# twosigma/Cook

Hardware: AMD Instinct MI355X
Metric: match-cycles/sec at 1M pending x 50k offers (higher is better)
Workload: dtype f64

## Files before the change

cook_amd/csrc/classfit_host.hpp:

```cpp

static int classfit_env() {
  static const int v = [] {
    const char* s = std::getenv("COOK_CLASSFIT");
    return s && (s[0] == '0' || s[0] == '1') ? s[0] - '0' : -1;
  }();
  return v;
}
static bool classfit_by_default(const cook_engine* e) {
  const int f = classfit_env();
  if (f >= 0) return f == 1;
  return g_engines_on_device[e->device & 63].load() >= 6;
}
static size_t cf_lds_bytes_host(unsigned NP, unsigned M, bool eq, unsigned G, unsigned S) {
  size_t n = sizeof(CfFixed) + (size_t)NP * 10u;
  n = (n + 7u) & ~(size_t)7u;
  if (eq) n += (size_t)M * 8u;
  n += ((size_t)G + 1u) * 2u + (size_t)G * 2u + (size_t)S * 2u;
  return n + 64u;
}
bool cf_setup(cook_engine* e, const MatchIn& in, const MatchIn* in_dev, const MatchState& st, const JobRec* jr, const JobCons* jcons, const OfferA* oa, const OfferB* ob,
              CfPoolCtx& ctx) {
  const unsigned K = in.K, M = in.M, G = in.G;
  e->cf_inelig = 0x10000u;
  if (K == 0 || M == 0 || M > CF_SORT_N || G > CF_MAXG || in.good_enough < 1.0 || in.has_x || in.reserved_bits || in.host_dup) return false;
  if (e->cf_max_host == 0xFFFFFFFFu || (size_t)e->cf_max_host > 8u * (size_t)M + 65536u) return false;
  CfBuf b{};
  b.ctl = e->cf_ctl.ensure(1);
  b.jr = jr, b.jcons = jcons, b.oa = oa, b.ob = ob;
  b.attr8 = e->cf_attr8.ensure(M);
  b.max_host = e->cf_max_host;
  b.h2o = e->cf_h2o.ensure((size_t)b.max_host + 1u);
  b.pos_fc = e->cf_pos[0].ensure(M), b.pos_fm = e->cf_pos[1].ensure(M), b.pos_cid = e->cf_pos[2].ensure(M);
  b.scr_fc = e->cf_scr[0].ensure(M), b.scr_fm = e->cf_scr[1].ensure(M), b.scr_cid = e->cf_scr[2].ensure(M);
  b.jobs = e->cf_jobs.ensure(K);
  b.gcount = e->cf_gcount.ensure(std::max(1u, G));
  b.gmem = e->cf_gmem.ensure((size_t)std::max(1u, G) * CF_GMEM);
  static_assert(sizeof(CfCtl) % 4 == 0, "cf_init clears the control block word by word");
  KM<cf_init, 256>(e, "cf_init", std::min(div_up(b.max_host + 1u, 1024u), 512u), b, b.max_host + 1u, std::max(1u, G));
  KM<cf_scan, 256>(e, "cf_scan", div_up(std::max(K, M), 256), in_dev, b, K, M);
  KM<cf_prepare, 1024>(e, "cf_prepare", 1u, in_dev, b, st.jmin, K, M, G, in.host_dup, in.reserved_bits ? 1u : 0u);
  KM<cf_pack_jobs, 256>(e, "cf_pack_jobs", div_up(K, 256), in_dev, b, K);
  static_assert(offsetof(CfCtl, t) <= 512, "the control block's head is read back through the 512-byte scratch");
  pinned_copy(e, e->h_scratch, b.ctl, offsetof(CfCtl, t), hipMemcpyDeviceToHost);
  sync(e);
  CfCtl hc;
  std::memcpy((void*)&hc, e->h_scratch, offsetof(CfCtl, t));
  e->cf_inelig = hc.inelig;
  if (hc.inelig) return false;
  const unsigned NP = (M + 63u) & ~63u;
  const unsigned S = hc.any_group ? e->cf_group_run_total + hc.n_grouped : 0u;
  if (cf_lds_bytes_host(NP, M, hc.any_eq != 0u, hc.any_group ? G : 0u, S) > CF_LDS_BYTES || S > 60000u) {
    e->cf_inelig = CF_X_SHAPE;
    return false;
  }
  ctx.in = in_dev;
  ctx.st = st;
  ctx.b = b;
  return true;
}
static void cf_prof_print(const uint32_t* q) {
#ifdef CF_PROF
  std::fprintf(stderr, "CFPROF (x16 shader cycles) decider: slow steps %u (candidates %u evaluation %u commit %u) plain steps %u in %u walk-total %u | class wave 1: poll %u answer %u answers %u idle %u idles %u | class wave 2: poll %u answer %u answers %u idle %u idles %u | walk ticks(100MHz) %u | batch boundaries: decider %u, batches without a walked job %u\n", q[27], q[24], q[25], q[26], q[28], q[29], q[31], q[32], q[33], q[35], q[36], q[37], q[40], q[41], q[43], q[44], q[45], q[CFS_TICKS_WALK], q[30], q[38]);
  std::fprintf(stderr, "CFPROF plain steps %u, C++ steps %u; steps that left the plain form: gpu kind %u, novel hosts %u, group %u, answer missing after the re-reads %u, guard band %u, epoch end %u\n", q[46], q[47], q[34] & 65535u, q[34] >> 16, q[39] & 65535u, q[39] >> 16, q[42] & 65535u, q[42] >> 16);
#else
  (void)q;
#endif
}
void cf_run(cook_engine* lead, cook_engine* const* es, unsigned n, hipStream_t stream) {
  cook_engine* e = lead;
  for (unsigned i0 = 0; i0 < n; i0 += (unsigned)CF_PACK) {
    const unsigned c = std::min<unsigned>(CF_PACK, n - i0);
    CfPack pk{};
    for (unsigned x = 0; x < (unsigned)CF_PACK; ++x) pk.c[x] = es[i0 + (x < c ? x : 0u)]->placement.walk;
    KLS("cf_walk", stream, cf_walk, c, CF_THREADS, pk);
  }
  for (unsigned i = 0; i < n; ++i) {
    const CfPoolCtx& c = es[i]->placement.walk;
    const unsigned G = es[i]->last_in.G;
    if (G) KLS("cf_group_chains", stream, cf_group_chains, div_up(G, 256), 256, c.b, c.st, G);
  }
  constexpr size_t SLOT = 16 + 48 * 4;
  if (!lead->h_cf) COOK_HIP(hipHostMalloc((void**)&lead->h_cf, 64 * SLOT, hipHostMallocDefault));
  for (unsigned i = 0; i < n; ++i) {
    char* slot = lead->h_cf + i * SLOT;
    COOK_HIP(hipMemcpyAsync(slot, es[i]->placement.walk.st.summary, 16, hipMemcpyDeviceToHost, stream));
    COOK_HIP(hipMemcpyAsync(slot + 16, es[i]->placement.walk.b.ctl->stats, 48 * 4, hipMemcpyDeviceToHost, stream));
  }
  COOK_HIP(hipStreamSynchronize(stream));
  for (unsigned i = 0; i < n; ++i) {
    cook_engine* x = es[i];
    const unsigned* sum = (const unsigned*)(lead->h_cf + i * SLOT);
    if (sum[3] == 0xDEADu) lead->fail(COOK_E_STATE, "cf_walk: the pool's tables do not fit the workgroup's LDS (the host's check let it through)");
    std::memcpy(x->cf_stats, lead->h_cf + i * SLOT + 16, 48 * 4);
    cf_prof_print(x->cf_stats);
    WinCtl c{};
    c.matched = sum[0], c.head_matched = sum[1], c.rounds = sum[2], c.head = x->last_in.K, c.visited_sum = x->cf_stats[CFS_WALKED];
    c.t_seq = x->cf_stats[CFS_TICKS_TOTAL], c.t_setup = x->cf_stats[CFS_TICKS_PROLOGUE];
    x->placement_complete(3, c);
  }
}
```

cook_amd/csrc/classfit_walk.hpp:

```cpp
#pragma once
#if defined(CF_PROF) && !defined(CF_STATS)
#define CF_STATS 1
#endif
#ifdef CF_STATS
#define CF_STAT(x) x
#define CF_TICKS() cook_ticks()
#else
#define CF_STAT(x) ((void)0)
#define CF_TICKS() 0ull
#endif
#ifdef CF_PROF
#define CF_PROF_T(x) const unsigned long long x = __builtin_readcyclecounter()
#define CF_PROF_ADD(i, d) prof[i] += (unsigned long long)(d)
#define CF_PROF_WHY(n) why = why == 3u ? (n) : why
#define CF_PROF_LEAVE() (why < 4u ? leave_a += 1ull << (16u * why) : leave_b += 1ull << (16u * (why - 4u)))
#else
#define CF_PROF_T(x) ((void)0)
#define CF_PROF_ADD(i, d) ((void)0)
#define CF_PROF_WHY(n) ((void)0)
#define CF_PROF_LEAVE() ((void)0)
#endif

#ifndef CF_AHEAD
#define CF_AHEAD 10
#endif
constexpr unsigned CF_BOARD = CF_AHEAD;
#ifndef CF_SLOTS_N
#define CF_SLOTS_N 12
#endif
constexpr unsigned CF_SLOTS = CF_SLOTS_N;
static_assert(CF_BOARD + 2u <= CF_SLOTS, "a slot is free again before its wave writes it two rows on");
static_assert(CF_SLOTS == 12u || CF_SLOTS == 24u, "cf_slot and classfit_asm.hpp know these two");
static __device__ __forceinline__ unsigned cf_slot(unsigned ord) { return ord - CF_SLOTS * ((ord * 43u) >> (CF_SLOTS == 12u ? 9 : 10)); }
constexpr unsigned CF_OVL = 58;
constexpr unsigned CF_EPOCH_AT = COOK_SHAPE(58, 8);
constexpr unsigned CFW_BOOKS = 4;
enum : unsigned { CFM_EXACT = 1u, CFM_EPOCH = 2u, CFM_BATCH_END = 3u };
enum : unsigned { CFX_NEXT_BASE = 0, CFX_SPARE1, CFX_LOGN, CFX_LOG_APPLIED, CFX_WALK_LO, CFX_WALK_HI, CFX_EX_LANE, CFX_FMAX_LO, CFX_FMAX_HI, CFX_EPOCH, CFX_MATCH_LO, CFX_MATCH_HI,
                  CFX_B1_LO, CFX_B1_HI, CFX_OVN, CFX_MINFC, CFX_MINFM, CFX_N = 24 };
constexpr uint32_t CF_ENT_NONE = 0x80000000u, CF_ENT_AMB = 0x40000000u;

struct __attribute__((aligned(8))) CfFree {
  uint32_t c, m;
};
struct CfEnt {
  uint32_t tag, pad, pos, cid;
  uint32_t fc, fm;
  double fa;
};
struct CfLog {
  uint32_t info, pos;
  uint32_t ofc, ofm, nfc, nfm, pad0, pad1;
};
struct CfPost {
  double fa;
  uint32_t w0;
  uint32_t pos;
  uint32_t fc, fm, cls, aux;
};
struct CfJobU {
  unsigned c, m, kind, L, n_eq, n_nov, grouped, grp, eq0, eq1, nov0, nov1;
};
struct CfLds {
  CfFree* fcm;
  uint16_t* cid;
  CfEnt* board;
  CfLog* log;
  uint32_t* ctrl;
  uint64_t* attr8;
  uint16_t *goff, *gcnt, *gids;
  CfJob* ring;
  CfPost* post2;
  CfClass* cls;
  uint32_t* pw;
  uint32_t* aw;
  uint32_t* gk;
  uint32_t* ovt;
  uint32_t* ovl;
  uint32_t* ckept;
  uint32_t* misc;
  const uint32_t* t;
  const uint32_t* envw;
};

struct CfLv8 {
  uint32_t v0, v1, v2, v3, v4, v5, v6, v7;
};
#define CF_FOR8(F) F(0) F(1) F(2) F(3) F(4) F(5) F(6) F(7)
static __device__ __forceinline__ unsigned cf_level_of(const uint32_t* t, uint32_t fc) {
  unsigned n = 0;
#pragma unroll
// ... 269 lines not shown
  constexpr bool is_decider = ROLE == 0, is_class_wave = ROLE == 1, is_books = ROLE == 2;
  const unsigned tid = threadIdx.x, lane = lane_id();
  CfCtl* ctl = b.ctl;
  const unsigned K = wave_uniform_u32(S.envw[CFE_K]), cmin = wave_uniform_u32(S.envw[CFE_CMIN]), mmin = wave_uniform_u32(S.envw[CFE_MMIN]);
  const uint32_t* t = S.t;
  CfLv8 tl = CfLv8{0u, 0u, 0u, 0u, 0u, 0u, 0u, 0u};
  if (is_class_wave) tl = cf_levels_load(t);
#define n_cls wave_uniform_u32(S.envw[CFE_NCLS])
#define n_kind wave_uniform_u32(S.envw[CFE_NKIND])
#define NP wave_uniform_u32(S.envw[CFE_NP])
  CfChunkLane c;
  unsigned nch_wave = 0;
  cf_setup_chunks(S.cls, n_cls, is_class_wave ? lw : 0xFFu, lane, c, nch_wave);
  c.lv = CfLv8{0u, 0u, 0u, 0u, 0u, 0u, 0u, 0u}, c.la = c.lv;
  unsigned my_kinds = 0;
  {
    const unsigned forw = is_class_wave ? lw : (is_decider && lane >= CF_OVL ? lane - CF_OVL + 1u : 0xFFu);
    for (unsigned ci = 0; ci < n_cls; ++ci)
      if (S.cls[ci].wave == forw && S.cls[ci].kind < 32u) my_kinds |= 1u << S.cls[ci].kind;
  }
  const unsigned wk = is_class_wave ? wave_uniform_u32(my_kinds) : 0u;
  unsigned one_cls = 0xFFFFFFFFu, u_off = 0, u_n = 0;
  double u_hTc = 0.0, u_hTm = 0.0;
  auto class_setup = [&] {
    unsigned cnt = 0, ci0 = 0;
    for (unsigned ci = 0; ci < n_cls; ++ci)
      if (S.cls[ci].wave == lw) ++cnt, ci0 = ci;
    one_cls = cnt == 1u ? ci0 : 0xFFFFFFFFu;
    const CfClass* cl = &S.cls[ci0];
    u_off = cl->off, u_n = cl->n, u_hTc = cl->hTc, u_hTm = cl->hTm;
  };
  if (is_class_wave) {
    class_setup();
    for (unsigned ch = 0; ch < nch_wave; ++ch) cf_tighten(S, tl, lane, ch, c);
    if (rep == 0u && lw != 0u) cf_wave_tables(S, lw, lane, c, wk, n_kind);
  }
  CfOvLane o;
  o.valid = 0u, o.id = 0u, o.cls = 0u, o.fc = 0u, o.fm = 0u, o.hTc = 0.0, o.hTm = 0.0;
  unsigned nrm = 0, rm1 = 0xFFFFFFFFu, rm2 = 0xFFFFFFFFu;
  unsigned minfc_all = wave_uniform_u32(S.envw[CFE_MINFC]), minfm_all = wave_uniform_u32(S.envw[CFE_MINFM]);
  unsigned matched = 0, head = 0;
  unsigned jc = 0, jm = 0, jmeta = 0, jgrp = 0, jeq0 = 0, jeq1 = 0, jnov0 = 0, jnov1 = 0;
  int res = -1;
  unsigned long long b1m = 0ull;
  unsigned seen = 0, gen = 0;
  unsigned tight_applied = 0;
  bool bk_room0 = false, nx_room0 = false, nx_walk = false;
  unsigned st_scans = 0, st_exact = 0, st_open = 0, st_ovwin = 0, st_gpu = 0, st_epochs = 0, st_tight = 0, st_walked = 0, st_dead = 0, st_opendead = 0, st_spins = 0, st_flips = 0,
           st_rewinds = 0;
  unsigned long long tk_epoch = 0, tk_books = 0, tk_walk = 0, tk_phase1 = 0;
#ifdef CF_PROF
  unsigned long long prof[8] = {0, 0, 0, 0, 0, 0, 0, 0}, bnd0 = 0ull;
  unsigned long long leave_a = 0ull, leave_b = 0ull;
#endif
  auto job_of = [&](unsigned s) -> CfJobU {
    CfJobU J;
    J.c = (unsigned)wave_read_lane((int)jc, (int)s), J.m = (unsigned)wave_read_lane((int)jm, (int)s);
    const unsigned meta = (unsigned)wave_read_lane((int)jmeta, (int)s);
    J.kind = meta & 255u, J.L = (meta >> 8) & 15u, J.n_eq = (meta >> 12) & 15u, J.n_nov = (meta >> 16) & 15u, J.grouped = (meta >> 20) & 1u;
    J.grp = 0u, J.eq0 = J.eq1 = 0u, J.nov0 = J.nov1 = 0xFFFFFFFFu;
    if (meta >> 12) {
      J.grp = (unsigned)wave_read_lane((int)jgrp, (int)s), J.eq0 = (unsigned)wave_read_lane((int)jeq0, (int)s), J.eq1 = (unsigned)wave_read_lane((int)jeq1, (int)s),
      J.nov0 = (unsigned)wave_read_lane((int)jnov0, (int)s), J.nov1 = (unsigned)wave_read_lane((int)jnov1, (int)s);
    }
    return J;
  };
  auto tables_room_any = [&](unsigned L, unsigned m) -> bool {
    bool r = S.ovt[L] > m;
    for (unsigned x = 1; x <= (unsigned)CF_CW; ++x) r = r || S.aw[x * CF_LV + L] > m;
    return r;
  };
  auto tables_walk = [&](unsigned kind, unsigned L, unsigned m) -> bool {
    bool r = false;
    if (kind == 0u) {
      r = S.ovt[L] > m;
      for (unsigned x = 1; x <= (unsigned)CF_CW; ++x) r = r || S.pw[x * CF_LV + L] > m;
    } else if (kind < (unsigned)CF_MAXKIND) {
      r = S.gk[kind * CF_LV + L] > m;
    }
    return r;
  };
  CfJob nxt;
  nxt.c = nxt.m = nxt.meta = nxt.grp = nxt.eq[0] = nxt.eq[1] = nxt.nov[0] = nxt.nov[1] = 0u;
  constexpr unsigned CF_PRE = 3;
  CfJob pre[CF_PRE];
  auto books_next = [&](unsigned nbase) -> unsigned long long {
    const unsigned nn = nbase < K ? cf_min(64u, K - nbase) : 0u;
    const unsigned nslot = (nbase >> 6) & 1u;
    const bool in = lane < nn;
    if (in) S.ring[nslot * 64u + lane] = nxt;
    const unsigned kind = nxt.meta & 255u, L = (nxt.meta >> 8) & 15u;
    nx_room0 = in && tables_room_any(L, nxt.m);
    nx_walk = in && tables_walk(kind, L, nxt.m);
    const unsigned long long wm = __ballot(nx_walk);
    if (lane == 0)
      S.misc[CFX_WALK_LO] = (unsigned)wm, S.misc[CFX_WALK_HI] = (unsigned)(wm >> 32), S.misc[CFX_LOGN] = 0u, S.misc[CFX_LOG_APPLIED] = 0u,
      S.ctrl[1] = wm ? (unsigned)__ffsll(wm) - 1u : 0u;
    return wm;
  };
  auto books_advance = [&](unsigned nbase) {
    nxt = pre[0];
#pragma unroll
    for (unsigned i = 0; i + 1u < CF_PRE; ++i) pre[i] = pre[i + 1u];
    if (nbase + 64u * (CF_PRE + 1u) + lane < K) pre[CF_PRE - 1u] = b.jobs[nbase + 64u * (CF_PRE + 1u) + lane];
  };
  __syncthreads();
  if (is_books) {
    if (lane < cf_min(64u, K)) nxt = b.jobs[lane];
    books_next(0u);
    bk_room0 = nx_room0;
    if (64u + lane < K) nxt = b.jobs[64u + lane];
#pragma unroll
    for (unsigned i = 0; i < CF_PRE; ++i) {
      pre[i] = nxt;
      if (64u * (i + 2u) + lane < K) pre[i] = b.jobs[64u * (i + 2u) + lane];
    }
  }
  if (is_decider) cook_set_prio_high();
  const unsigned long long t_loop = cook_ticks();
  __syncthreads();
  const bool isov = lane < CF_OVL;
  const unsigned clw = isov ? 0u : lane - CF_OVL + 1u;

  for (unsigned base = 0; base < K;) {
    const unsigned bn = cf_min(64u, K - base);
    const unsigned slot = (base >> 6) & 1u;
    const unsigned long long walkmask = wave_uniform_u64((unsigned long long)S.misc[CFX_WALK_LO] | (unsigned long long)S.misc[CFX_WALK_HI] << 32);
    const unsigned nw = (unsigned)__popcll(walkmask);
    st_walked += nw;
    if (!is_books) {
      const CfJob j = S.ring[slot * 64u + (lane < bn ? lane : 0u)];
      const bool in = lane < bn;
      jc = in ? j.c : 0u, jm = in ? j.m : 0u, jmeta = in ? j.meta : CF_KIND_NONE, jgrp = j.grp, jeq0 = j.eq[0], jeq1 = j.eq[1], jnov0 = j.nov[0], jnov1 = j.nov[1];
    }
    res = -1;
    if (is_decider) b1m = __ballot(!(jc <= minfc_all && jm <= minfm_all));
    unsigned logn = 0;
    unsigned long long todo = walkmask;
    unsigned cur_ord = 0;
    unsigned ph = 0;
    bool batch_done = nw == 0u;
    auto decider_books = [&](unsigned n_placed) {
      if (lane < bn) st.job_to_offer[base + lane] = res;
      const unsigned long long mm = __ballot(res >= 0);
      if (base == 0u) head = (unsigned)(mm & 1ull);
      const bool live = isov && o.valid != 0u;
      const unsigned nl = live ? cf_level_of(t, o.fc) : 0u;
#define CF_OV_T(i) unsigned v##i = nl > (unsigned)i ? o.fm + 1u : 0u;
      CF_FOR8(CF_OV_T)
#undef CF_OV_T
      wave_max8_u32(v0, v1, v2, v3, v4, v5, v6, v7);
      if (lane == 0) {
        S.misc[CFX_MATCH_LO] = (unsigned)mm, S.misc[CFX_MATCH_HI] = (unsigned)(mm >> 32), S.misc[CFX_B1_LO] = (unsigned)b1m, S.misc[CFX_B1_HI] = (unsigned)(b1m >> 32);
        S.misc[CFX_LOGN] = n_placed, S.misc[CFX_MINFC] = minfc_all, S.misc[CFX_MINFM] = minfm_all;
#define CF_OV_S(i) S.ovt[i] = v##i;
        CF_FOR8(CF_OV_S)
#undef CF_OV_S
      }
    };
    const unsigned long long tw0 = CF_TICKS();
    CF_PROF_T(cw0);
// ... 6 lines not shown
      if (is_decider) {
#if COOK_HAS_ASM_WALK
        cf_u32x16 ST = {0u, 0u, 0u, 0u, 0u, 0u, 0u, 0u, 0u, 0u, 0u, 0u, 0u, 0u, 0u, 0u};
        const unsigned a_board = wave_uniform_u32(cook_lds_off(S.board)), a_log = wave_uniform_u32(cook_lds_off(S.log));
        cf_u32x8 JB = {jc, jm, jmeta, a_board + clw * (unsigned)sizeof(CfEnt), lane, jeq0, jeq1, a_board};
        const unsigned long long rel0 = cook_ballot(!isov & ((my_kinds & 1u) != 0u)), ovm = cf_below(CF_OVL);
        auto st_pack = [&] {
          const unsigned long long hc = (unsigned long long)__double_as_longlong(o.hTc), hm = (unsigned long long)__double_as_longlong(o.hTm);
          ST[0] = o.valid, ST[1] = o.id, ST[2] = (unsigned)hc, ST[3] = (unsigned)(hc >> 32), ST[4] = (unsigned)hm, ST[5] = (unsigned)(hm >> 32), ST[6] = o.cls, ST[7] = o.fc, ST[8] = o.fm,
          ST[9] = nrm, ST[10] = rm1, ST[11] = rm2, ST[12] = (unsigned)res, ST[13] = a_log + logn * (unsigned)sizeof(CfLog);
        };
        auto st_unpack = [&] {
          o.valid = ST[0], o.id = ST[1], o.hTc = __longlong_as_double((long long)((unsigned long long)ST[3] << 32 | ST[2])),
          o.hTm = __longlong_as_double((long long)((unsigned long long)ST[5] << 32 | ST[4])), o.cls = ST[6], o.fc = ST[7], o.fm = ST[8], nrm = ST[9], rm1 = ST[10], rm2 = ST[11],
          res = (int)ST[12];
        };
#endif
        while (md == 0u) {
          todo = wave_uniform_u64(todo), cur_ord = wave_uniform_u32(cur_ord), logn = wave_uniform_u32(logn), matched = wave_uniform_u32(matched), gen = wave_uniform_u32(gen);
          minfc_all = wave_uniform_u32(minfc_all), minfm_all = wave_uniform_u32(minfm_all), b1m = wave_uniform_u64(b1m);
#if COOK_HAS_ASM_WALK
          if (todo != 0ull) {
            st_pack();
            CF_PROF_T(f0);
#define CF_U(x) wave_uniform_u32((unsigned)(x))
            cf_u32x8 SC = {CF_U(matched), CF_U(minfc_all), CF_U(b1m), CF_U(b1m >> 32), CF_U(minfm_all), 1u, CF_U(todo), CF_U(todo >> 32)};
            cf_u32x8 AR = {0u, 0u, CF_U(cf_slot(cur_ord) * 8u * (unsigned)sizeof(CfEnt)), 0u, 0u, CF_U(cmin), CF_U(mmin), a_board};
            cf_u32x8 MK = {CF_U(rel0), CF_U(rel0 >> 32), CF_U(ovm), CF_U(ovm >> 32), CF_U(cook_lds_off(S.attr8)), CF_U(cur_ord), 0u, CF_U(base << 12 | (gen & 15u) << 8)};
            asm volatile(CF_ASM_DECIDER_RUN
                         : "+{v[64:79]}"(ST), "+{s[36:43]}"(SC), "+{s[44:51]}"(AR), "+{s[52:59]}"(MK)
                         : "{v[80:87]}"(JB)
                         : "v88", "v89", "v90", "v91", "v92", "v93", "v94", "v95", "v96", "v97", "v98", "v99", "v100", "v101", "v102", "v103", "v104", "v105", "v106", "v107", "v108",
                           "v109", "v110", "v111", "v112", "v113", "v114", "v115", "v116", "v117", "v118", "v119", "s60", "s61", "s62", "s63", "s64", "s65", "s66", "s67", "s68", "s69",
                           "s70", "s71", "s72", "s73", "s74", "s75", "s76", "s77", "s78", "s79", "s80", "s81", "s82", "s83", "s84", "s85", "s86", "vcc", "scc", "memory");
            matched = CF_U(SC[0]), minfc_all = CF_U(SC[1]), minfm_all = CF_U(SC[4]);
            b1m = wave_uniform_u64((unsigned long long)SC[3] << 32 | SC[2]);
            todo = wave_uniform_u64((unsigned long long)SC[7] << 32 | SC[6]);
            logn = (CF_U(ST[13]) - a_log) / (unsigned)sizeof(CfLog);
            CF_PROF_ADD(4, CF_U(MK[5]) - cur_ord);
            cur_ord = CF_U(MK[5]);
#undef CF_U
            CF_PROF_T(f1);
            CF_PROF_ADD(5, f1 - f0);
            WAIT_LDS();
            st_unpack();
          }
#endif
          if (todo == 0ull) {
#ifdef CF_PROF
            bnd0 = __builtin_readcyclecounter();
#endif
            decider_books(logn);
            md = CFM_BATCH_END;
            st_lane0_b32(&S.ctrl[0], md);
            break;
          }
          CF_PROF_T(p0);
          const unsigned s = (unsigned)__ffsll(todo) - 1u;
          const unsigned ord = cur_ord;
          st_lane0_b32(&S.ctrl[1], s | ord << 8);
          const unsigned Jc = (unsigned)wave_read_lane((int)jc, (int)s), Jm = (unsigned)wave_read_lane((int)jm, (int)s), meta = (unsigned)wave_read_lane((int)jmeta, (int)s);
          const unsigned kind = meta & 255u;
          const unsigned want = (base + s) << 12 | (gen & 15u) << 8;
#ifdef CF_PROF
          unsigned why = kind != 0u ? 0u : ((meta >> 16) & 15u) ? 1u : ((meta >> 20) & 1u) ? 2u : 3u;
#endif
          const CfEnt* e = &S.board[cf_slot(ord) * 8u + clw];
          const bool relevant = !isov && kind < 32u && ((my_kinds >> (kind & 31u)) & 1u);
          unsigned cpos, ccid, cfc, cfm;
          double cfa;
          bool acc;
          bool ok_ov = isov & (o.valid != 0u) & (kind == 0u) & (o.fc >= Jc) & (o.fm >= Jm);
          if (meta >> 12) {
            const CfJobU J = job_of(s);
            ok_ov = ok_ov & cf_cons_ok(S, J, o.id, ok_ov);
          }
          for (;;) {
            const unsigned t1 = ld_wg(&e->tag);
            COMPILER_FENCE();
            cpos = e->pos, ccid = e->cid, cfc = e->fc, cfm = e->fm, cfa = e->fa;
            COMPILER_FENCE();
            const unsigned t2 = ld_wg(&e->tag);
            const unsigned behind = (nrm - t1) & 255u, p = cpos & 0xFFFFu;
            const bool ours = (t1 == t2) & ((t1 & ~255u) == want);
            acc = ours & (((ccid & CF_ENT_NONE) != 0u) | ((behind <= 2u) & (p != rm1) & (p != rm2)));
            if (cook_ballot(relevant & !acc) == 0ull) break;
            for (unsigned long long rq = cook_ballot(relevant & !acc & ours); rq != 0ull; rq &= rq - 1ull) {
              const unsigned L = (unsigned)__ffsll(rq) - 1u;
              const unsigned xid = (unsigned)wave_read_lane((int)(ccid & CF_IDMASK), (int)L);
              if (cook_ballot(ok_ov & (o.id == xid)) != 0ull && lane == L) acc = true, ccid = CF_ENT_NONE;
            }
            if (cook_ballot(relevant & !acc) == 0ull) break;
            CF_STAT(++st_spins);
            SPIN_PAUSE_NEAR();
          }
          CF_PROF_T(p1);
          CF_PROF_ADD(0, p1 - p0);
          const unsigned vfc = isov ? o.fc : cfc, vfm = isov ? o.fm : cfm, vid = isov ? o.id : (ccid & CF_IDMASK);
          const bool vvalid = isov ? (o.valid != 0u && kind == 0u) : (relevant && !(ccid & CF_ENT_NONE));
          const bool room = vvalid & (vfc >= Jc) & (vfm >= Jm);
          const bool ok = isov ? ok_ov : room;
          double fov = 1.0 - ((double)(vfc - Jc) * o.hTc + (double)(vfm - Jm) * o.hTm);
          OPAQUE_V(fov);
          const double fa = ok ? (isov ? fov : cfa) : 0.0;
          const float ff = (float)fa;
          const float mx = wave_max_f32(ff);
          const unsigned long long eqm = cook_ballot(ok & (ff == mx)), nearm = cook_ballot(ok & (ff >= mx - CF_BAND32)),
                                   ambm = cook_ballot(ok & !isov & ((ccid & CF_ENT_AMB) != 0u) & (ff >= mx - CF_BAND32));
          CF_PROF_T(p2);
          CF_PROF_ADD(1, p2 - p1);
          CF_PROF_ADD(3, 1);
          if (!(mx > 0.0f)) {
            CF_PROF_LEAVE();
            todo &= todo - 1ull, ++cur_ord;
            continue;
          }
          unsigned l0 = (unsigned)__ffsll(eqm) - 1u;
          if ((nearm & (nearm - 1ull)) != 0ull || ambm != 0ull) {
            CF_PROF_WHY(4u);
            const unsigned long long mxb = wave_max_u64((unsigned long long)__double_as_longlong(fa));
            const double f0 = __longlong_as_double((long long)mxb);
            l0 = (unsigned)__ffsll(__ballot(ok && (unsigned long long)__double_as_longlong(fa) == mxb)) - 1u;
            const unsigned long long near = __ballot(ok && fa >= f0 - CF_BAND);
            const bool amb = (near & (near - 1ull)) != 0ull || (__ballot(ok && !isov && (ccid & CF_ENT_AMB) && fa >= f0 - CF_BAND) != 0ull);
            if (amb) {
              md = CFM_EXACT;
              if (lane == 0) S.misc[CFX_EX_LANE] = s, S.misc[CFX_FMAX_LO] = (unsigned)mxb, S.misc[CFX_FMAX_HI] = (unsigned)(mxb >> 32), st_wg(&S.ctrl[0], md);
              CF_PROF_LEAVE();
              break;
            }
          }
          todo &= todo - 1ull, ++cur_ord;
          const unsigned ofc = (unsigned)wave_read_lane((int)vfc, (int)l0), ofm = (unsigned)wave_read_lane((int)vfm, (int)l0), id = (unsigned)wave_read_lane((int)vid, (int)l0);
          const unsigned nfc = ofc - Jc, nfm = ofm - Jm;
          const bool dead = nfc < cmin || nfm < mmin;
          const bool from_ov = l0 < CF_OVL;
          ++matched;
          res = lane == s ? (int)id : res;
          b1m |= cook_ballot((jc > nfc) | (jm > nfm)) & ~cf_below(s) & ~(1ull << s);
          minfc_all = cf_min(minfc_all, nfc), minfm_all = cf_min(minfm_all, nfm);
          unsigned lpos = 0, linfo = s;
          if (from_ov) {
            CF_STAT(++st_ovwin);
            const bool me = lane == l0;
            o.fc = me ? nfc : o.fc, o.fm = me ? nfm : o.fm, o.valid = (me && dead) ? 0u : o.valid;
            if (dead) CF_STAT(++st_dead);
          } else {
            const bool gpu_place = kind != 0u;
            const unsigned pos = (unsigned)wave_read_lane((int)cpos, (int)l0);
            const unsigned cls2 = ((unsigned)wave_read_lane((int)ccid, (int)l0) >> 16) & 255u;
            const unsigned cw = l0 - CF_OVL + 1u;
            const unsigned cnt2 = (unsigned)wave_read_lane((int)nrm, (int)l0) + 1u;
            lpos = pos & 0xFFFFu, linfo = s | cw << 8 | (pos >> 16) << 12 | (gpu_place ? 1u : 0u) << 20;
            if (gpu_place) {
              st_lane0_b64(&S.fcm[lpos], nfc, nfm);
              if (lane == 0) S.cid[lpos] = (uint16_t)(S.cid[lpos] | CF_OCC);
              CF_STAT(++st_gpu);
            } else {
              st_lane0_b64(&S.fcm[lpos], 0u, 0u);
            }
            st_lane0_b32(&S.ctrl[1u + cw], cnt2);
            const bool me = lane == l0;
            rm2 = me ? rm1 : rm2, rm1 = me ? lpos : rm1, nrm = me ? cnt2 : nrm;
            if (!gpu_place && !dead) {
              CF_STAT(++st_open);
              const unsigned long long vm = cook_ballot(isov & (o.valid != 0u));
              const unsigned lf = (unsigned)__ffsll(~(vm | ~cf_below(CF_OVL))) - 1u;
              const CfClass* cl = &S.cls[cls2];
              const double hTc2 = cl->hTc, hTm2 = cl->hTm;
              const bool nl = lane == lf;
              o.valid = nl ? 1u : o.valid, o.id = nl ? id : o.id, o.cls = nl ? cls2 : o.cls, o.fc = nl ? nfc : o.fc, o.fm = nl ? nfm : o.fm, o.hTc = nl ? hTc2 : o.hTc,
              o.hTm = nl ? hTm2 : o.hTm;
              const unsigned live1 = wave_uniform_u32((unsigned)__popcll(vm) + 1u);
              if (live1 >= CF_EPOCH_AT) md = CFM_EPOCH;
            } else if (!gpu_place) {
              CF_STAT(++st_opendead);
            }
          }
          st_lane0_b128(&S.log[logn].info, linfo, lpos, ofc, ofm);
          ++logn;
          if ((meta >> 20) & 1u) {
            const unsigned grp = (unsigned)wave_read_lane((int)jgrp, (int)s);
            if (lane == 0) {
              const unsigned g0 = S.goff[grp], gn = S.gcnt[grp];
              S.gids[g0 + gn] = (uint16_t)id;
              COMPILER_FENCE();
              st_wg(&S.gcnt[grp], (uint16_t)(gn + 1u));
            }
            wave_sync();
          }
          md = wave_uniform_u32(md);
          if (md == CFM_EPOCH) {
            CF_PROF_WHY(5u);
            if (lane == 0) S.misc[CFX_EX_LANE] = s, S.misc[CFX_LOGN] = logn, st_wg(&S.ctrl[0], md);
          }
          CF_PROF_LEAVE();
          CF_PROF_T(p3);
          CF_PROF_ADD(2, p3 - p2);
        }
      } else if (is_class_wave) {
        while (md == 0u) {
#if COOK_HAS_ASM_WALK
          if (one_cls != 0xFFFFFFFFu) {
            const cf_u32x8 LV = {c.lv.v0, c.lv.v1, c.lv.v2, c.lv.v3, c.lv.v4, c.lv.v5, c.lv.v6, c.lv.v7};
            const cf_u32x8 JC = {jc, jm, jmeta, lane, 0u, 0u, 0u, 0u};
#define CF_U(x) wave_uniform_u32((unsigned)(x))
            const unsigned long long hcb = (unsigned long long)__double_as_longlong(u_hTc), hmb = (unsigned long long)__double_as_longlong(u_hTm);
            const cf_u32x8 AR = {CF_U(cook_lds_off(S.board)), CF_U(lw), CF_U(base), CF_U((gen & 15u) << 8), CF_U(u_off), CF_U(u_n), CF_U(cook_lds_off(S.cid)), CF_U(one_cls << 16)};
            const cf_u32x8 A2 = {CF_U(hcb), CF_U(hcb >> 32), CF_U(hmb), CF_U(hmb >> 32), CF_U(rep), CF_U(nrep), CF_U(S.cls[one_cls].kind), CF_BOARD};
            for (;;) {
              cf_u32x8 SC = {CF_U(todo), CF_U(todo >> 32), CF_U(cur_ord), CF_U(ph), CF_U(seen), 3u, 0u, 0u};
              asm volatile(CF_ASM_CLASS_STEP
                           : "+{s[36:43]}"(SC)
                           : "{v[64:71]}"(LV), "{v[72:79]}"(JC), "{s[44:51]}"(AR), "{s[52:59]}"(A2)
                           : "v80", "v81", "v82", "v83", "v84", "v85", "v86", "v87", "v88", "v89", "v90", "v91", "v92", "v93", "v94", "v95", "v96", "v97", "v98", "v99", "s60", "s61", "s62",
                             "s63", "s64", "s65", "s66", "s67", "s68", "s69", "s70", "s71", "s72", "s73", "s74", "s75", "s76", "s77", "s78", "s79", "s80", "s81", "s82", "s83", "vcc", "scc",
                             "memory");
              todo = wave_uniform_u64((unsigned long long)SC[1] << 32 | SC[0]), cur_ord = wave_uniform_u32(SC[2]), ph = wave_uniform_u32(SC[3]);
              const unsigned status = wave_uniform_u32(SC[5]);
              if (status == 0u) continue;
              if (status == 2u) {
                SPIN_PAUSE_NEAR();
                continue;
              }
              break;
            }
#undef CF_U
            WAIT_LDS();
          }
#endif
          CF_PROF_T(q0);
          unsigned mode, hw, cnt;
          {
            const unsigned a0 = ld_wg(&S.ctrl[0]), a1 = ld_wg(&S.ctrl[1]), a2 = ld_wg(&S.ctrl[1u + lw]);
            mode = (unsigned)wave_read_lane((int)a0, 0), hw = (unsigned)wave_read_lane((int)a1, 0), cnt = (unsigned)wave_read_lane((int)a2, 0);
          }
          if (mode != 0u) {
            md = mode;
            break;
          }
          COMPILER_FENCE();
          auto answer = [&](unsigned s, unsigned ord, bool again) {
            const unsigned Jc = (unsigned)wave_read_lane((int)jc, (int)s), Jm = (unsigned)wave_read_lane((int)jm, (int)s), meta = (unsigned)wave_read_lane((int)jmeta, (int)s);
            const unsigned kind = meta & 255u;
            if (!(kind < 32u && ((wk >> kind) & 1u))) return;
            CF_PROF_T(q1);
#ifdef CF_DELAY_C
// ... 44 lines not shown
                  CF_STAT(++st_scans);
                }
              }
            }
            if (!done) {
              const CfJobU J = job_of(s);
              CfAns a;
              cf_class_answer(S, tl, J, lane, c, a, st_scans, st_tight);
              const unsigned long long fb = (unsigned long long)__double_as_longlong(a.fa);
              st_lane0_b32(&e->tag, 0xFFFFFFFFu);
              st_lane0_b128(&e->fc, a.fc, a.fm, (unsigned)fb, (unsigned)(fb >> 32));
              st_lane0_b64(&e->pos, a.pos | a.ch << 16, a.have ? (a.cid | a.cls << 16 | (a.amb ? CF_ENT_AMB : 0u)) : CF_ENT_NONE);
              st_lane0_b32(&e->tag, tag);
            }
            CF_PROF_T(q2);
            CF_PROF_ADD(0, q1 - q0);
            CF_PROF_ADD(1, q2 - q1);
            CF_PROF_ADD(3, 1);
          };
          if (cnt != seen) {
            seen = cnt;
            CF_STAT(++st_rewinds);
            unsigned long long t2 = walkmask & ~cf_below(hw & 255u);
            unsigned o2 = hw >> 8, p2 = o2;
            while (p2 >= nrep) p2 -= nrep;
            for (; t2 != 0ull && o2 < cur_ord; t2 &= t2 - 1ull, ++o2, p2 = p2 + 1u == nrep ? 0u : p2 + 1u)
              if (p2 == rep && wk != 0u) answer((unsigned)__ffsll(t2) - 1u, o2, true);
          }
          if (cur_ord < (hw >> 8)) {
            todo = walkmask & ~cf_below(hw & 255u);
            cur_ord = hw >> 8;
            ph = cur_ord;
            while (ph >= nrep) ph -= nrep;
          }
          while (todo != 0ull && ph != rep) {
            todo &= todo - 1ull, ++cur_ord;
            ph = ph + 1u == nrep ? 0u : ph + 1u;
          }
          if (todo != 0ull && wk != 0u && cur_ord < (hw >> 8) + CF_BOARD) {
            const unsigned s = (unsigned)__ffsll(todo) - 1u;
            const unsigned ord = cur_ord;
            todo &= todo - 1ull, ++cur_ord;
            ph = ph + 1u == nrep ? 0u : ph + 1u;
            answer(s, ord, false);
            continue;
          }
          if (wk != 0u) SPIN_PAUSE_NEAR();
          else SPIN_PAUSE_IDLE();
          CF_PROF_T(q4);
          CF_PROF_ADD(4, q4 - q0);
          CF_PROF_ADD(5, 1);
        }
      } else {
        while (md == 0u) {
          const unsigned mode = cf_poll(&S.ctrl[0]);
          if (mode != 0u) {
            md = mode;
            break;
          }
          SPIN_PAUSE_IDLE();
        }
      }
      EMU_SITE("classfit: collective");
      WAIT_LDS();
      __syncthreads();
      md = wave_uniform_u32(md);
      if (md == CFM_BATCH_END) {
        batch_done = true;
        if (tid == 0) st_wg(&S.ctrl[0], 0u);
        if (is_class_wave) seen = cf_poll(&S.ctrl[1u + lw]);
        break;
      }
      bool epoch = md == CFM_EPOCH;
      const unsigned s = wave_uniform_u32(S.misc[CFX_EX_LANE]);
      if (md == CFM_EXACT) {
        ++st_exact;
        const double fmax = __longlong_as_double((long long)((unsigned long long)S.misc[CFX_FMAX_LO] | (unsigned long long)S.misc[CFX_FMAX_HI] << 32));
        CfPost mine;
        if (is_decider) {
          const CfJobU J = job_of(s);
          cf_overlay_query_exact(S, J, lane, o, fmax, cf_pow2(-(int)wave_uniform_u32(S.envw[CFE_KC])), cf_pow2(-(int)wave_uniform_u32(S.envw[CFE_KM])), mine);
          if (lane == 0) S.post2[0] = mine;
        } else if (is_class_wave && rep == 0u && lw != 0u) {
          const CfJobU J = job_of(s);
          cf_class_query_exact(S, J, lane, c, fmax, cf_pow2(-(int)wave_uniform_u32(S.envw[CFE_KC])), cf_pow2(-(int)wave_uniform_u32(S.envw[CFE_KM])), mine, st_scans);
          if (lane == 0) S.post2[lw] = mine;
        }
        EMU_SITE("classfit: exact turn");
        __syncthreads();
        if (is_decider) {
          const CfJobU J = job_of(s);
          unsigned used_sets = 0;
          for (unsigned ci = 0; ci < n_cls; ++ci) used_sets |= 1u << wave_uniform_u32(S.cls[ci].wave);
          const CfVerdict v = cf_verdict_exact(S.post2, lane, used_sets);
          const unsigned nfc = v.fc - J.c, nfm = v.fm - J.m;
          const bool dead = nfc < cmin || nfm < mmin;
          const bool from_ov = v.src == 0;
          const bool gpu_place = !from_ov && J.kind != 0u;
          const bool opens = !from_ov && !gpu_place && !dead;
          ++matched;
          if (lane == s) res = (int)v.id;
          b1m |= __ballot((jc > nfc) | (jm > nfm)) & ~cf_below(s) & ~(1ull << s);
          minfc_all = cf_min(minfc_all, nfc), minfm_all = cf_min(minfm_all, nfm);
          unsigned live = (unsigned)__popcll(__ballot(isov && o.valid != 0u));
          unsigned lpos = 0, linfo = s;
          if (from_ov) {
            CF_STAT(++st_ovwin);
            if (lane == v.pos) {
              o.fc = nfc, o.fm = nfm;
              if (dead) o.valid = 0u;
            }
            if (dead) --live;
          } else {
            lpos = v.pos, linfo = s | (unsigned)v.src << 8 | v.aux << 12 | (gpu_place ? 1u : 0u) << 20;
            if (lane == CF_OVL - 1u + (unsigned)v.src) {
              if (gpu_place) S.fcm[lpos] = CfFree{nfc, nfm}, S.cid[lpos] = (uint16_t)(S.cid[lpos] | CF_OCC);
              else S.fcm[lpos] = CfFree{0u, 0u};
              ++nrm, rm2 = rm1, rm1 = lpos;
// ... 140 lines not shown
          class_setup();
          for (unsigned ch = 0; ch < nch_wave; ++ch) cf_tighten(S, tl, lane, ch, c);
          if (rep == 0u && lw != 0u) cf_wave_tables(S, lw, lane, c, wk, n_kind);
          tight_applied = st_tight;
        }
        if (tid == 0) S.misc[CFX_LOG_APPLIED] = S.misc[CFX_LOGN];
        tk_epoch += CF_TICKS() - te;
      }
      {
        ++gen;
        if (is_class_wave) {
          todo = walkmask & ~cf_below(s) & ~(1ull << s), cur_ord = (unsigned)__popcll(walkmask & cf_below(s)) + 1u;
          ph = cur_ord;
          while (ph >= nrep) ph -= nrep;
        }
      }
      if (tid == 0) st_wg(&S.ctrl[0], 0u);
      EMU_SITE("classfit: collective done");
      __syncthreads();
      if (is_class_wave) seen = cf_poll(&S.ctrl[1u + lw]);
    }
    tk_walk += CF_TICKS() - tw0;
    CF_PROF_T(cw1);
    CF_PROF_ADD(7, cw1 - cw0);
    const unsigned long long tp0 = CF_TICKS();
    if (is_decider && nw == 0u) decider_books(0u);
    if (nw != 0u) {
      if (is_class_wave) {
        const CfLog* lp = &S.log[lane];
        const unsigned info = lp->info, ofc = lp->ofc, ofm = lp->ofm;
        const unsigned n_log = wave_uniform_u32(S.misc[CFX_LOGN]), a0 = wave_uniform_u32(S.misc[CFX_LOG_APPLIED]);
        const bool mine = lane >= a0 && lane < n_log && ((info >> 8) & 15u) == lw;
        const unsigned ch = (info >> 12) & 63u;
        const unsigned nl = cf_level_of(tl, ofc);
#define CF_LV_AT(i) const unsigned g##i = (unsigned)__shfl((int)c.lv.v##i, (int)ch, COOK_WAVE);
        CF_FOR8(CF_LV_AT)
#undef CF_LV_AT
        bool was_max = ((info >> 20) & 1u) != 0u;
#define CF_WAS_MAX(i) was_max = was_max | (((unsigned)i < nl) & (g##i == ofm + 1u));
        CF_FOR8(CF_WAS_MAX)
#undef CF_WAS_MAX
        unsigned long long stale = 0ull;
        for (unsigned long long fm = cook_ballot(mine & was_max); fm != 0ull; fm &= fm - 1ull) stale |= 1ull << (unsigned)wave_read_lane((int)ch, __ffsll(fm) - 1);
        bool dirty = st_tight != tight_applied;
        for (; stale != 0ull; stale &= stale - 1ull) {
          cf_tighten(S, tl, lane, (unsigned)__ffsll(stale) - 1u, c);
          ++st_tight;
          dirty = true;
        }
        if (dirty && rep == 0u && lw != 0u) cf_wave_tables(S, lw, lane, c, wk, n_kind);
        tight_applied = st_tight;
      }
    }
    EMU_SITE("classfit: phase 2");
    __syncthreads();
    tk_phase1 += CF_TICKS() - tp0;
    if (is_books) {
      const unsigned long long tb0 = CF_TICKS();
      const unsigned long long mm = (unsigned long long)S.misc[CFX_MATCH_LO] | (unsigned long long)S.misc[CFX_MATCH_HI] << 32,
                               bb = (unsigned long long)S.misc[CFX_B1_LO] | (unsigned long long)S.misc[CFX_B1_HI] << 32;
      const unsigned n_log = wave_uniform_u32(S.misc[CFX_LOGN]);
      const CfJob j = S.ring[slot * 64u + (lane < bn ? lane : 0u)];
      const bool unm = lane < bn && !((mm >> lane) & 1ull);
      const unsigned L = (j.meta >> 8) & 15u;
      bool room = unm && tables_room_any(L, j.m);
      const bool flip = unm && !room && bk_room0 && n_log != 0u;
      if (__ballot(flip) != 0ull) {
        ++st_flips;
        for (unsigned x = 0; x < n_log; ++x) {
          const CfLog lg = S.log[x];
          if (flip && (lg.info & 255u) > lane && lg.ofc >= j.c && lg.ofm >= j.m) room = true;
        }
      }
      if (lane < bn && st.fail_code) {
        unsigned fail = 0u;
        if (unm) {
          fail = (((bb >> lane) & 1ull) ? 1u : 0u) | (room ? 2u : 0u);
          if (fail == 0u) fail = 8u;
        }
        st.fail_code[base + lane] = fail;
      }
      unsigned nb = base + 64u;
      unsigned long long nwm = books_next(nb);
      const unsigned minfc_pub = wave_uniform_u32(S.misc[CFX_MINFC]), minfm_pub = wave_uniform_u32(S.misc[CFX_MINFM]);
      while (nb < K && nwm == 0ull) {
        if (nb + lane < K) {
          st.job_to_offer[nb + lane] = -1;
          if (st.fail_code) {
            const unsigned fail = ((nxt.c > minfc_pub || nxt.m > minfm_pub) ? 1u : 0u) | (nx_room0 ? 2u : 0u);
            st.fail_code[nb + lane] = fail != 0u ? fail : 8u;
          }
        }
        books_advance(nb);
        nb += 64u;
        nwm = books_next(nb);
      }
      if (lane == 0) S.misc[CFX_NEXT_BASE] = nb;
      bk_room0 = nx_room0;
      books_advance(nb);
      tk_books += CF_TICKS() - tb0;
    }
    EMU_SITE("classfit: batch end");
    __syncthreads();
    const unsigned nbase = wave_uniform_u32(S.misc[CFX_NEXT_BASE]);
#ifdef CF_PROF
    if (is_class_wave) prof[6] += 16ull * ((nbase - base) / 64u - 1u);
#endif
    base = nbase;
  }
  if (is_decider) {
    if (lane == 0) {
      st.summary[0] = matched;
      st.summary[1] = (matched == 0u || head) ? 1u : 0u;
      st.summary[2] = st_epochs;
      const unsigned long long t_end = cook_ticks();
      uint32_t* sx = ctl->stats;
      sx[CFS_MATCHED] = matched, sx[CFS_OV_WIN] = st_ovwin, sx[CFS_OPEN] = st_open, sx[CFS_OPEN_DEAD] = st_opendead, sx[CFS_GPU_PLACE] = st_gpu, sx[CFS_EPOCHS] = st_epochs,
      sx[CFS_EXACT] = st_exact, sx[CFS_WALKED] = st_walked, sx[CFS_DEAD_DROP] = st_dead, sx[CFS_BATCHES] = (K + 63u) / 64u, sx[CFS_PRESETTLED] = K - st_walked;
      sx[CFS_TICKS_TOTAL] = (uint32_t)(t_end - t_start), sx[CFS_TICKS_PROLOGUE] = (uint32_t)(t_loop - t_start), sx[CFS_TICKS_EPOCH] = (uint32_t)tk_epoch;
      sx[CFS_TICKS_WALK] = (uint32_t)tk_walk, sx[CFS_TICKS_PHASE1] = (uint32_t)tk_phase1;
      sx[CFS_HWID_DECIDER] = cook_hw_id();
    }
    const unsigned sp = wave_max_u32(!isov ? st_spins : 0u);
    if (lane == 0) ctl->stats[CFS_SPINS] = sp;
  }
  if (is_class_wave && lane == 0) atomicAdd(&ctl->stats[CFS_SCANS], st_scans), atomicAdd(&ctl->stats[CFS_TIGHTEN], st_tight), atomicAdd(&ctl->stats[CFS_REWINDS], st_rewinds);
  if (is_books && lane == 0) ctl->stats[CFS_TICKS_PRECHECK] = (uint32_t)tk_books, ctl->stats[CFS_FLIPS] = st_flips, ctl->stats[CFS_HWID_BOOKS] = cook_hw_id();
#ifdef CF_PROF
  if (lane == 0 && (is_decider || (is_class_wave && lw >= 1u && lw <= 2u && rep == 0u)))
    for (int i = 0; i < 8; ++i)
      if (is_decider || (i != 2 && i != 7 && !(lw == 2u && i == 6))) ctl->stats[24 + 8 * (is_decider ? 0u : lw) + i] = (uint32_t)(prof[i] >> 4);
  if (lane == 0 && is_decider)
    ctl->stats[34] = (uint32_t)leave_a, ctl->stats[39] = (uint32_t)(leave_a >> 32), ctl->stats[42] = (uint32_t)leave_b, ctl->stats[46] = (uint32_t)prof[4], ctl->stats[47] = (uint32_t)prof[3];
#endif
#undef n_cls
#undef n_kind
#undef NP
}

static __device__ __forceinline__ void cf_walk_pool(char* lds, const MatchIn* __restrict__ inp, const MatchState& st, const CfBuf& b) {
  const unsigned tid = threadIdx.x, lane = lane_id(), w = wave_id();
  CfCtl* ctl = b.ctl;
  const unsigned K = inp->K, M = ctl->M, G = inp->G;
  const unsigned NP = (M + 63u) & ~63u;
  const unsigned long long t_start = cook_ticks();
  const bool any_eq = ctl->any_eq != 0u, any_group = ctl->any_group != 0u;
  __shared__ unsigned s_total, s_wsum[CF_WAVES];
  static_assert(CF_MAXG % CF_THREADS == 0, "the groups are dealt out GPT to a thread: a workgroup size that does not divide CF_MAXG would leave some without one");
  constexpr unsigned GPT = CF_MAXG / CF_THREADS;
  unsigned gsz[GPT];
  unsigned gsum = 0;
#pragma unroll
  for (unsigned x = 0; x < GPT; ++x) {
    const unsigned g = tid * GPT + x;
    unsigned sz = 0;
    if (any_group && g < G && b.gcount[g] != 0u) sz = (inp->g_run_off ? inp->g_run_off[g + 1] - inp->g_run_off[g] : 0u) + b.gcount[g];
    gsz[x] = sz, gsum += sz;
  }
  unsigned incl = gsum;
  for (unsigned d = 1; d < 64u; d <<= 1) {
    const unsigned y = shfl_up_t<unsigned>(incl, d);
    if (lane >= d) incl += y;
  }
  if (lane == 63u) s_wsum[w] = incl;
  __syncthreads();
  unsigned wbase = 0;
  for (unsigned x = 0; x < w; ++x) wbase += s_wsum[x];
  if (tid == CF_THREADS - 1) s_total = wbase + incl;
  __syncthreads();
  const unsigned Stot = any_group ? s_total : 0u, Gl = any_group ? G : 0u;
  CfLds S;
  {
    CfFixed* F = (CfFixed*)lds;
    S.board = F->board, S.log = F->log, S.ring = F->ring, S.post2 = F->post2, S.cls = F->cls, S.pw = F->pw, S.aw = F->aw, S.gk = F->gk, S.ovt = F->ovt, S.ctrl = F->ctrl, S.ovl = F->ovl,
    S.ckept = F->ckept, S.misc = F->misc, S.t = F->env_t, S.envw = F->envw;
    char* p = lds + sizeof(CfFixed);
    S.fcm = (CfFree*)p, p += NP * 8u;
    S.cid = (uint16_t*)p, p += NP * 2u;
    p = lds + (((unsigned)(p - lds) + 7u) & ~7u);
    S.attr8 = (uint64_t*)p;
    if (any_eq) p += M * 8u;
    S.goff = (uint16_t*)p, p += (Gl + 1u) * 2u;
    S.gcnt = (uint16_t*)p, p += Gl * 2u;
    S.gids = (uint16_t*)p, p += Stot * 2u;
    if ((unsigned)(p - lds) > CF_LDS_BYTES) {
      if (tid == 0) atomicOr(&ctl->inelig, (unsigned)CF_X_SHAPE), st.summary[3] = 0xDEADu;
      return;
// ... 95 lines not shown
```

Measured before the change: 23.45.

## Drop books-wave spin on mode word; precompute per-level room tables across lanes

The books wave no longer spin-polls the control word before the collective barrier. It reads a new mode slot in LDS after the barrier, which the decider writes before raising the mode. The per-level room and walk maxima over the class waves' tables are now reduced once per batch into lane registers and fetched with shuffles, replacing per-lane loops of LDS reads. Books-phase LDS reads are also hoisted before the phase-2 barrier when the wave is otherwise idle. Together these aim to cut spin traffic and LDS latency on the books wave's critical path, at the cost of extra registers and a dependence on the mode slot being written before every barrier.

```diff
diff --git a/cook_amd/csrc/classfit_host.hpp b/cook_amd/csrc/classfit_host.hpp
--- a/cook_amd/csrc/classfit_host.hpp
+++ b/cook_amd/csrc/classfit_host.hpp
@@ -60,7 +60,7 @@
 }
 static void cf_prof_print(const uint32_t* q) {
 #ifdef CF_PROF
-  std::fprintf(stderr, "CFPROF (x16 shader cycles) decider: slow steps %u (candidates %u evaluation %u commit %u) plain steps %u in %u walk-total %u | class wave 1: poll %u answer %u answers %u idle %u idles %u | class wave 2: poll %u answer %u answers %u idle %u idles %u | walk ticks(100MHz) %u | batch boundaries: decider %u, batches without a walked job %u\n", q[27], q[24], q[25], q[26], q[28], q[29], q[31], q[32], q[33], q[35], q[36], q[37], q[40], q[41], q[43], q[44], q[45], q[CFS_TICKS_WALK], q[30], q[38]);
+  std::fprintf(stderr, "CFPROF (x16 shader cycles) decider: slow steps %u (candidates %u evaluation %u commit %u) plain steps %u in %u walk-total %u | class wave 1: poll %u answer %u answers %u idle %u idles %u | class wave 2: poll %u answer %u answers %u | decider, mode word raised -> barrier left: %u over %u turns | walk ticks(100MHz) %u | batch boundaries: decider %u, batches without a walked job %u\n", q[27], q[24], q[25], q[26], q[28], q[29], q[31], q[32], q[33], q[35], q[36], q[37], q[40], q[41], q[43], q[44], q[45], q[CFS_TICKS_WALK], q[30], q[38]);
   std::fprintf(stderr, "CFPROF plain steps %u, C++ steps %u; steps that left the plain form: gpu kind %u, novel hosts %u, group %u, answer missing after the re-reads %u, guard band %u, epoch end %u\n", q[46], q[47], q[34] & 65535u, q[34] >> 16, q[39] & 65535u, q[39] >> 16, q[42] & 65535u, q[42] >> 16);
 #else
   (void)q;
diff --git a/cook_amd/csrc/classfit_walk.hpp b/cook_amd/csrc/classfit_walk.hpp
--- a/cook_amd/csrc/classfit_walk.hpp
+++ b/cook_amd/csrc/classfit_walk.hpp
@@ -36,7 +36,7 @@
 constexpr unsigned CF_EPOCH_AT = COOK_SHAPE(58, 8);
 constexpr unsigned CFW_BOOKS = 4;
 enum : unsigned { CFM_EXACT = 1u, CFM_EPOCH = 2u, CFM_BATCH_END = 3u };
-enum : unsigned { CFX_NEXT_BASE = 0, CFX_SPARE1, CFX_LOGN, CFX_LOG_APPLIED, CFX_WALK_LO, CFX_WALK_HI, CFX_EX_LANE, CFX_FMAX_LO, CFX_FMAX_HI, CFX_EPOCH, CFX_MATCH_LO, CFX_MATCH_HI,
+enum : unsigned { CFX_NEXT_BASE = 0, CFX_MODE, CFX_LOGN, CFX_LOG_APPLIED, CFX_WALK_LO, CFX_WALK_HI, CFX_EX_LANE, CFX_FMAX_LO, CFX_FMAX_HI, CFX_EPOCH, CFX_MATCH_LO, CFX_MATCH_HI,
                   CFX_B1_LO, CFX_B1_HI, CFX_OVN, CFX_MINFC, CFX_MINFM, CFX_N = 24 };
 constexpr uint32_t CF_ENT_NONE = 0x80000000u, CF_ENT_AMB = 0x40000000u;
 
@@ -412,6 +412,11 @@
 #ifdef CF_PROF
   unsigned long long prof[8] = {0, 0, 0, 0, 0, 0, 0, 0}, bnd0 = 0ull;
   unsigned long long leave_a = 0ull, leave_b = 0ull;
+  unsigned long long rz0 = 0ull, rz_sum = 0ull;
+  unsigned rz_n = 0;
+#define CF_PROF_RAISE() rz0 = __builtin_readcyclecounter()
+#else
+#define CF_PROF_RAISE() ((void)0)
 #endif
   auto job_of = [&](unsigned s) -> CfJobU {
     CfJobU J;
@@ -425,19 +430,20 @@
     }
     return J;
   };
-  auto tables_room_any = [&](unsigned L, unsigned m) -> bool {
-    bool r = S.ovt[L] > m;
-    for (unsigned x = 1; x <= (unsigned)CF_CW; ++x) r = r || S.aw[x * CF_LV + L] > m;
-    return r;
+  uint32_t row_a = 0u, row_p = 0u;
+  auto tables_reduce = [&] {
+    const unsigned l7 = lane & (unsigned)(CF_LV - 1);
+    const uint32_t ov = S.ovt[l7];
+    uint32_t a = ov, p = ov;
+#pragma unroll
+    for (unsigned x = 1; x <= (unsigned)CF_CW; ++x) a = cf_max(a, S.aw[x * CF_LV + l7]), p = cf_max(p, S.pw[x * CF_LV + l7]);
+    row_a = a, row_p = p;
   };
-  auto tables_walk = [&](unsigned kind, unsigned L, unsigned m) -> bool {
-    bool r = false;
-    if (kind == 0u) {
-      r = S.ovt[L] > m;
-      for (unsigned x = 1; x <= (unsigned)CF_CW; ++x) r = r || S.pw[x * CF_LV + L] > m;
-    } else if (kind < (unsigned)CF_MAXKIND) {
-      r = S.gk[kind * CF_LV + L] > m;
-    }
+  auto tables_room_any = [&](unsigned L, unsigned m) -> bool { return (uint32_t)__shfl((int)row_a, (int)(L & (unsigned)(CF_LV - 1)), COOK_WAVE) > m; };
+  auto tables_walk = [&](bool in, unsigned kind, unsigned L, unsigned m) -> bool {
+    const uint32_t p = (uint32_t)__shfl((int)row_p, (int)(L & (unsigned)(CF_LV - 1)), COOK_WAVE);
+    bool r = in && kind == 0u && p > m;
+    if (in && kind != 0u && kind < (unsigned)CF_MAXKIND) r = S.gk[kind * CF_LV + L] > m;
     return r;
   };
   CfJob nxt;
@@ -450,8 +456,9 @@
     const bool in = lane < nn;
     if (in) S.ring[nslot * 64u + lane] = nxt;
     const unsigned kind = nxt.meta & 255u, L = (nxt.meta >> 8) & 15u;
-    nx_room0 = in && tables_room_any(L, nxt.m);
-    nx_walk = in && tables_walk(kind, L, nxt.m);
+    const bool any = tables_room_any(L, nxt.m);
+    nx_room0 = in && any;
+    nx_walk = tables_walk(in, kind, L, nxt.m);
     const unsigned long long wm = __ballot(nx_walk);
     if (lane == 0)
       S.misc[CFX_WALK_LO] = (unsigned)wm, S.misc[CFX_WALK_HI] = (unsigned)(wm >> 32), S.misc[CFX_LOGN] = 0u, S.misc[CFX_LOG_APPLIED] = 0u,
@@ -467,6 +474,7 @@
   __syncthreads();
   if (is_books) {
     if (lane < cf_min(64u, K)) nxt = b.jobs[lane];
+    tables_reduce();
     books_next(0u);
     bk_room0 = nx_room0;
     if (64u + lane < K) nxt = b.jobs[64u + lane];
@@ -579,6 +587,8 @@
 #endif
             decider_books(logn);
             md = CFM_BATCH_END;
+            CF_PROF_RAISE();
+            st_lane0_b32(&S.misc[CFX_MODE], md);
             st_lane0_b32(&S.ctrl[0], md);
             break;
           }
@@ -652,7 +662,8 @@
             const bool amb = (near & (near - 1ull)) != 0ull || (__ballot(ok && !isov && (ccid & CF_ENT_AMB) && fa >= f0 - CF_BAND) != 0ull);
             if (amb) {
               md = CFM_EXACT;
-              if (lane == 0) S.misc[CFX_EX_LANE] = s, S.misc[CFX_FMAX_LO] = (unsigned)mxb, S.misc[CFX_FMAX_HI] = (unsigned)(mxb >> 32), st_wg(&S.ctrl[0], md);
+              CF_PROF_RAISE();
+              if (lane == 0) S.misc[CFX_EX_LANE] = s, S.misc[CFX_FMAX_LO] = (unsigned)mxb, S.misc[CFX_FMAX_HI] = (unsigned)(mxb >> 32), S.misc[CFX_MODE] = md, st_wg(&S.ctrl[0], md);
               CF_PROF_LEAVE();
               break;
             }
@@ -719,7 +730,8 @@
           md = wave_uniform_u32(md);
           if (md == CFM_EPOCH) {
             CF_PROF_WHY(5u);
-            if (lane == 0) S.misc[CFX_EX_LANE] = s, S.misc[CFX_LOGN] = logn, st_wg(&S.ctrl[0], md);
+            CF_PROF_RAISE();
+            if (lane == 0) S.misc[CFX_EX_LANE] = s, S.misc[CFX_LOGN] = logn, S.misc[CFX_MODE] = md, st_wg(&S.ctrl[0], md);
           }
           CF_PROF_LEAVE();
           CF_PROF_T(p3);
@@ -870,18 +882,14 @@
           CF_PROF_ADD(5, 1);
         }
       } else {
-        while (md == 0u) {
-          const unsigned mode = cf_poll(&S.ctrl[0]);
-          if (mode != 0u) {
-            md = mode;
-            break;
-          }
-          SPIN_PAUSE_IDLE();
-        }
       }
       EMU_SITE("classfit: collective");
       WAIT_LDS();
       __syncthreads();
+#ifdef CF_PROF
+      if (is_decider) rz_sum += __builtin_readcyclecounter() - rz0, ++rz_n;
+#endif
+      if (is_books) md = cf_poll(&S.misc[CFX_MODE]);
       md = wave_uniform_u32(md);
       if (md == CFM_BATCH_END) {
         batch_done = true;
@@ -1128,18 +1136,29 @@
         tight_applied = st_tight;
       }
     }
+    unsigned bk_m0 = 0, bk_m1 = 0, bk_b0 = 0, bk_b1 = 0, bk_nlog = 0, bk_minfc = 0, bk_minfm = 0;
+    CfJob bk_j;
+    bk_j.c = bk_j.m = bk_j.meta = bk_j.grp = bk_j.eq[0] = bk_j.eq[1] = bk_j.nov[0] = bk_j.nov[1] = 0u;
+    auto books_reads = [&] {
+      bk_m0 = S.misc[CFX_MATCH_LO], bk_m1 = S.misc[CFX_MATCH_HI], bk_b0 = S.misc[CFX_B1_LO], bk_b1 = S.misc[CFX_B1_HI], bk_nlog = S.misc[CFX_LOGN];
+      bk_minfc = S.misc[CFX_MINFC], bk_minfm = S.misc[CFX_MINFM];
+      bk_j = S.ring[slot * 64u + (lane < bn ? lane : 0u)];
+    };
+    if (is_books && nw != 0u) books_reads();
     EMU_SITE("classfit: phase 2");
     __syncthreads();
     tk_phase1 += CF_TICKS() - tp0;
     if (is_books) {
       const unsigned long long tb0 = CF_TICKS();
-      const unsigned long long mm = (unsigned long long)S.misc[CFX_MATCH_LO] | (unsigned long long)S.misc[CFX_MATCH_HI] << 32,
-                               bb = (unsigned long long)S.misc[CFX_B1_LO] | (unsigned long long)S.misc[CFX_B1_HI] << 32;
-      const unsigned n_log = wave_uniform_u32(S.misc[CFX_LOGN]);
-      const CfJob j = S.ring[slot * 64u + (lane < bn ? lane : 0u)];
+      if (nw == 0u) books_reads();
+      tables_reduce();
+      const unsigned long long mm = (unsigned long long)bk_m0 | (unsigned long long)bk_m1 << 32, bb = (unsigned long long)bk_b0 | (unsigned long long)bk_b1 << 32;
+      const unsigned n_log = wave_uniform_u32(bk_nlog);
+      const CfJob& j = bk_j;
       const bool unm = lane < bn && !((mm >> lane) & 1ull);
       const unsigned L = (j.meta >> 8) & 15u;
-      bool room = unm && tables_room_any(L, j.m);
+      const bool any = tables_room_any(L, j.m);
+      bool room = unm && any;
       const bool flip = unm && !room && bk_room0 && n_log != 0u;
       if (__ballot(flip) != 0ull) {
         ++st_flips;
@@ -1158,7 +1177,7 @@
       }
       unsigned nb = base + 64u;
       unsigned long long nwm = books_next(nb);
-      const unsigned minfc_pub = wave_uniform_u32(S.misc[CFX_MINFC]), minfm_pub = wave_uniform_u32(S.misc[CFX_MINFM]);
+      const unsigned minfc_pub = wave_uniform_u32(bk_minfc), minfm_pub = wave_uniform_u32(bk_minfm);
       while (nb < K && nwm == 0ull) {
         if (nb + lane < K) {
           st.job_to_offer[nb + lane] = -1;
@@ -1205,10 +1224,12 @@
 #ifdef CF_PROF
   if (lane == 0 && (is_decider || (is_class_wave && lw >= 1u && lw <= 2u && rep == 0u)))
     for (int i = 0; i < 8; ++i)
-      if (is_decider || (i != 2 && i != 7 && !(lw == 2u && i == 6))) ctl->stats[24 + 8 * (is_decider ? 0u : lw) + i] = (uint32_t)(prof[i] >> 4);
+      if (is_decider || (i != 2 && i != 7 && !(lw == 2u && i >= 4))) ctl->stats[24 + 8 * (is_decider ? 0u : lw) + i] = (uint32_t)(prof[i] >> 4);
   if (lane == 0 && is_decider)
-    ctl->stats[34] = (uint32_t)leave_a, ctl->stats[39] = (uint32_t)(leave_a >> 32), ctl->stats[42] = (uint32_t)leave_b, ctl->stats[46] = (uint32_t)prof[4], ctl->stats[47] = (uint32_t)prof[3];
-#endif
+    ctl->stats[34] = (uint32_t)leave_a, ctl->stats[39] = (uint32_t)(leave_a >> 32), ctl->stats[42] = (uint32_t)leave_b, ctl->stats[46] = (uint32_t)prof[4], ctl->stats[47] = (uint32_t)prof[3],
+    ctl->stats[44] = (uint32_t)(rz_sum >> 4), ctl->stats[45] = rz_n;
+#endif
+#undef CF_PROF_RAISE
 #undef n_cls
 #undef n_kind
 #undef NP
```

New measurement: 23.58 (median of 6 runs). Within noise of the previous version (+0.6%).
